# rsinghlab/GNN-Tumor-Seg

Hardware: AMD Instinct MI355X
Metric: supervoxel-graphs/sec training, 7xSAGE-pool-256, 15k-node graphs (higher is better)
Workload: dtype f32; 1 GPU; C2: 7xGraphSAGE-pool-256 (8 SAGEConv), fwd+weighted-CE+bwd+AdamW, 4 x 15000-node/86350-edge lattice graphs per GPU, 4-chan feat, fp32; global_batch=4, nodes_per_batch=60000, edges_per_batch=345400, parallelism=dp1

## Files before the change

### gnn-tumor-seg_amd/csrc/gts_narrow.hip

```cpp
#include "gts_gemm_skinny.h"

namespace gts {
namespace {

constexpr int kFirstW = 256, kFirstS = 4;

__global__ __launch_bounds__(kBlock) void first_layer_bwd_kernel(const float* __restrict__ g, const float* __restrict__ x,
                                                                const float* __restrict__ m0,
                                                                const float* __restrict__ w_neigh, float* __restrict__ gm,
                                                                float* __restrict__ part_x, float* __restrict__ part_m,
                                                                int64_t m, int64_t rows_per_chunk) {
  constexpr int W = kFirstW, S = kFirstS;
  __shared__ v4f red[kWavesPerBlock - 1][2 * S + 1][kWave];
  const int lane = threadIdx.x & (kWave - 1), rl = threadIdx.x / kWave;
  const int64_t row0 = blockIdx.x * rows_per_chunk, row1 = min(m, row0 + rows_per_chunk);
  v4f wn[S];
#pragma unroll
  for (int e = 0; e < 4; ++e) {
    const v4f t = *reinterpret_cast<const v4f*>(w_neigh + static_cast<size_t>(4 * lane + e) * S);
#pragma unroll
    for (int j = 0; j < S; ++j) wn[j][e] = t[j];
  }
  v4f ax[S + 1], am[S];
#pragma unroll
// ... 44 lines not shown
  }
  __syncthreads();
  if (rl != 0) return;
#pragma unroll
  for (int i = 0; i <= S; ++i) {
    v4f total = ax[i];
    for (int l = 1; l < kWavesPerBlock; ++l) total += red[l - 1][i][lane];
    *reinterpret_cast<v4f*>(part_x + (static_cast<size_t>(blockIdx.x) * (S + 1) + i) * W + 4 * lane) = total;
  }
#pragma unroll
  for (int i = 0; i < S; ++i) {
    v4f total = am[i];
    for (int l = 1; l < kWavesPerBlock; ++l) total += red[l - 1][S + 1 + i][lane];
    *reinterpret_cast<v4f*>(part_m + (static_cast<size_t>(blockIdx.x) * S + i) * W + 4 * lane) = total;
  }
}

inline bool first_layer_shape(int64_t m, int64_t w, int64_t s0, int64_t s1) {
  return m > 0 && m < (1LL << 31) && w == kFirstW && s0 == kFirstS && s1 == kFirstS;
}

constexpr int kTopK = 256, kTopC = 4;
constexpr int kCeRowsPerThread = 4, kCeRows = kBlock * kCeRowsPerThread;

__device__ __forceinline__ float top_label_weight(long long label, const float* __restrict__ class_w, bool* valid, int* y) {
  *valid = label >= 0 && label < kTopC;
  *y = *valid ? static_cast<int>(label) : 0;
  return !*valid ? 0.0f : (class_w != nullptr ? class_w[*y] : 1.0f);
}

__global__ __launch_bounds__(kBlock) void top_den_kernel(const int64_t* __restrict__ labels, const float* __restrict__ class_w,
                                                        float* __restrict__ ce_part, int64_t n) {
  __shared__ float red[kWavesPerBlock];
  float den = 0.f;
  const int64_t base = (static_cast<int64_t>(blockIdx.x) * kBlock + threadIdx.x) * kCeRowsPerThread;
  for (int r = 0; r < kCeRowsPerThread; ++r) {
    const int64_t i = base + r;
    if (i >= n) break;
    bool valid;
    int y;
    den += top_label_weight(labels[i], class_w, &valid, &y);
  }
  for (int s = kWave / 2; s >= 1; s >>= 1) den += __shfl_xor(den, s, kWave);
  const int lane = threadIdx.x & (kWave - 1), wave = threadIdx.x / kWave;
  if (lane == 0) red[wave] = den;
  __syncthreads();
  if (threadIdx.x == 0) ce_part[2 * blockIdx.x + 1] = (red[0] + red[1]) + (red[2] + red[3]);
}

__device__ __forceinline__ float lane_value(float v, int lane) {
  return __int_as_float(__builtin_amdgcn_readlane(__float_as_int(v), lane));
}

__global__ __launch_bounds__(kBlock) void top_layer_train_kernel(
    const float* __restrict__ h, const float* __restrict__ mx, const float* __restrict__ w_self,
    const float* __restrict__ w_neigh, const float* __restrict__ bias, const int64_t* __restrict__ labels,
    const float* __restrict__ class_w, const float* __restrict__ ce_part, int ce_blocks, float* __restrict__ logits,
    float* __restrict__ g, float* __restrict__ term, float* __restrict__ part_h, float* __restrict__ part_m,
    float* __restrict__ part_b, int64_t m, int64_t rows_per_chunk) {
  constexpr int W = kTopK, C = kTopC;
  __shared__ v4f red[kWavesPerBlock - 1][2 * C][kWave];
  __shared__ v4f colsum[kBlock];
  __shared__ float dred[kBlock];
  const int lane = threadIdx.x & (kWave - 1), rl = threadIdx.x / kWave;
  const int64_t row0 = blockIdx.x * rows_per_chunk, row1 = min(m, row0 + rows_per_chunk);
  colsum[threadIdx.x] = v4f{0.f, 0.f, 0.f, 0.f};
  float den = 0.f;
  if (ce_part != nullptr) {
    for (int b = threadIdx.x; b < ce_blocks; b += kBlock) den += ce_part[2 * b + 1];
    dred[threadIdx.x] = den;
    __syncthreads();
    for (int s = kBlock / 2; s >= 1; s >>= 1) {
      if (threadIdx.x < s) dred[threadIdx.x] += dred[threadIdx.x + s];
      __syncthreads();
    }
    den = dred[0];
  } else {
    __syncthreads();
  }
  v4f ws[C], wn[C];
#pragma unroll
  for (int n = 0; n < C; ++n) {
    ws[n] = *reinterpret_cast<const v4f*>(w_self + static_cast<size_t>(n) * W + 4 * lane);
    wn[n] = *reinterpret_cast<const v4f*>(w_neigh + static_cast<size_t>(n) * W + 4 * lane);
  }
  const v4f bv = *reinterpret_cast<const v4f*>(bias);
  v4f ah[C], am[C];
#pragma unroll
  for (int i = 0; i < C; ++i) ah[i] = am[i] = v4f{0.f, 0.f, 0.f, 0.f};
  const bool upper32 = (lane & 32) != 0, upper16 = (lane & 16) != 0;
  const int sel = lane & 3;
  auto dots = [&](const v4f fh, const v4f fm) __attribute__((always_inline)) {
    float d[C];
#pragma unroll
    for (int n = 0; n < C; ++n) {
      d[n] = 0.f;
#pragma unroll
      for (int e = 0; e < 4; ++e) d[n] = __builtin_fmaf(fh[e], ws[n][e], d[n]);
#pragma unroll
      for (int e = 0; e < 4; ++e) d[n] = __builtin_fmaf(fm[e], wn[n][e], d[n]);
    }
    const float keep0 = upper32 ? d[2] : d[0], keep1 = upper32 ? d[3] : d[1];
    const float send0 = upper32 ? d[0] : d[2], send1 = upper32 ? d[1] : d[3];
    const float a = keep0 + __shfl_xor(send0, 32, kWave), b = keep1 + __shfl_xor(send1, 32, kWave);
    float c = (upper16 ? b : a) + __shfl_xor(upper16 ? a : b, 16, kWave);
#pragma unroll
    for (int o = 8; o > 0; o >>= 1) c += __shfl_xor(c, o, kWave);
    return c;
  };
  constexpr int kAhead = 4;
  for (int64_t first = row0 + rl; first < row1; first += kAhead * kWavesPerBlock) {
    v4f fh[kAhead], fm[kAhead];
#pragma unroll
    for (int u = 0; u < kAhead; ++u) {
      const int64_t row = first + u * kWavesPerBlock < row1 ? first + u * kWavesPerBlock : first;
      fh[u] = *reinterpret_cast<const v4f*>(h + static_cast<size_t>(row) * W + 4 * lane);
      fm[u] = *reinterpret_cast<const v4f*>(mx + static_cast<size_t>(row) * W + 4 * lane);
    }
    const bool mine = first + sel * kWavesPerBlock < row1;
    const int64_t my_row = mine ? first + sel * kWavesPerBlock : first;
    const long long label = labels[my_row];
    float x[C];
#pragma unroll
    for (int n = 0; n < C; ++n) x[n] = 0.f;
#pragma unroll
    for (int u = 0; u < kAhead; ++u) {
      const float c = dots(fh[u], fm[u]);
#pragma unroll
      for (int n = 0; n < C; ++n) {
        const float t = lane_value(c, 16 * n);
        x[n] = sel == u ? t : x[n];
      }
    }
#pragma unroll
    for (int n = 0; n < C; ++n) x[n] = x[n] + bv[n];
    float v[C];
    float top = -INFINITY;
#pragma unroll
    for (int c = 0; c < C; ++c) v[c] = x[c], top = fmaxf(top, v[c]);
    float sum = 0.f;
#pragma unroll
    for (int c = 0; c < C; ++c) v[c] = expf(v[c] - top), sum += v[c];
    bool valid;
    int y;
    const float w = top_label_weight(label, class_w, &valid, &y);
    const float xy = y == 0 ? x[0] : y == 1 ? x[1] : y == 2 ? x[2] : x[3];
    const float loss_term = valid ? w * (logf(sum) + top - xy) : (label == -100 ? 0.0f : NAN);
    v4f gv;
#pragma unroll
    for (int c = 0; c < C; ++c) {
      const float gu = w * (v[c] / sum - (c == y ? 1.0f : 0.0f));
      gv[c] = ce_part != nullptr ? gu / den : gu;
    }
    if (lane < kAhead && mine) {
      *reinterpret_cast<v4f*>(logits + static_cast<size_t>(my_row) * C) = v4f{x[0], x[1], x[2], x[3]};
      *reinterpret_cast<v4f*>(g + static_cast<size_t>(my_row) * C) = gv;
      term[my_row] = loss_term;
      const int slot = static_cast<int>((my_row - row0) & (kBlock - 1));
      colsum[slot] += 1.0f * gv;
    }
#pragma unroll
    for (int u = 0; u < kAhead; ++u) {
      if (first + u * kWavesPerBlock < row1) {
#pragma unroll
        for (int i = 0; i < C; ++i) {
          const float s = lane_value(gv[i], u);
          ah[i] += s * fh[u];
          am[i] += s * fm[u];
        }
      }
    }
  }
  if (rl > 0) {
#pragma unroll
    for (int i = 0; i < C; ++i) red[rl - 1][i][lane] = ah[i], red[rl - 1][C + i][lane] = am[i];
  }
  __syncthreads();
  if (rl != 0) return;
#pragma unroll
  for (int i = 0; i < C; ++i) {
    v4f total = ah[i];
    for (int l = 1; l < kWavesPerBlock; ++l) total += red[l - 1][i][lane];
    *reinterpret_cast<v4f*>(part_h + (static_cast<size_t>(blockIdx.x) * C + i) * W + 4 * lane) = total;
  }
#pragma unroll
  for (int i = 0; i < C; ++i) {
    v4f total = am[i];
    for (int l = 1; l < kWavesPerBlock; ++l) total += red[l - 1][C + i][lane];
    *reinterpret_cast<v4f*>(part_m + (static_cast<size_t>(blockIdx.x) * C + i) * W + 4 * lane) = total;
  }
  if (lane == 0) {
    const int live = static_cast<int>(min(static_cast<int64_t>(kBlock), row1 - row0));
    v4f total = colsum[0];
    for (int l = 1; l < live; ++l) total += colsum[l];
    *reinterpret_cast<v4f*>(part_b + static_cast<size_t>(blockIdx.x) * C) = total;
  }
}

__global__ __launch_bounds__(kBlock) void top_loss_kernel(const float* __restrict__ term, float* __restrict__ ce_part, int64_t n) {
  __shared__ float red[kWavesPerBlock];
  float num = 0.f;
  const int64_t base = (static_cast<int64_t>(blockIdx.x) * kBlock + threadIdx.x) * kCeRowsPerThread;
  if (base + kCeRowsPerThread <= n) {
    const v4f t = *reinterpret_cast<const v4f*>(term + base);
#pragma unroll
    for (int r = 0; r < kCeRowsPerThread; ++r) num += t[r];
  } else {
    for (int r = 0; r < kCeRowsPerThread; ++r) {
      if (base + r >= n) break;
      num += term[base + r];
    }
  }
  for (int s = kWave / 2; s >= 1; s >>= 1) num += __shfl_xor(num, s, kWave);
  const int lane = threadIdx.x & (kWave - 1), wave = threadIdx.x / kWave;
  if (lane == 0) red[wave] = num;
  __syncthreads();
  if (threadIdx.x == 0) ce_part[2 * blockIdx.x] = (red[0] + red[1]) + (red[2] + red[3]);
}

constexpr int kTopSumGroups = kTopC * kTopK / 16;

__global__ __launch_bounds__(kBlock) void top_finish_kernel(const float* __restrict__ part_h, const float* __restrict__ part_m,
// ... 62 lines not shown
  return t;
}

}
}

extern "C" int64_t gts_sage_first_layer_bwd_workspace(int64_t m, int64_t w, int64_t s0, int64_t s1) {
  using namespace gts;
  if (!first_layer_shape(m, w, s0, s1)) return 0;
  return static_cast<int64_t>(kSkinnyChunks) * (s0 + 1 + s1) * w * static_cast<int64_t>(sizeof(float));
}

extern "C" int32_t gts_sage_first_layer_bwd_f32(const float* g, const float* x, const float* m0, const float* w_neigh,
                                                float* gm, float* gw_self, float* g_bias, float* gw_neigh,
                                                float* workspace, int64_t workspace_bytes, int64_t m, int64_t w,
                                                int64_t s0, int64_t s1, void* stream) {
  using namespace gts;
  if (!g || !x || !m0 || !w_neigh || !gm || !gw_self || !g_bias || !gw_neigh || !workspace) return GTS_ERR_NULL;
  if (!first_layer_shape(m, w, s0, s1)) return GTS_ERR_SHAPE;
  if (workspace_bytes < gts_sage_first_layer_bwd_workspace(m, w, s0, s1)) return GTS_ERR_SHAPE;
  hipStream_t st = static_cast<hipStream_t>(stream);
  const int64_t rpc = (m + kSkinnyChunks - 1) / kSkinnyChunks;
  const int chunks = static_cast<int>((m + rpc - 1) / rpc);
  const int W = kFirstW, S = kFirstS;
  float* part_x = workspace;
  float* part_m = workspace + static_cast<size_t>(chunks) * (S + 1) * W;
  first_layer_bwd_kernel<<<chunks, kBlock, 0, st>>>(g, x, m0, w_neigh, gm, part_x, part_m, m, rpc);
  skinny_sum_kernel<<<((S + 1) * W + 15) / 16, kBlock, 0, st>>>(part_x, gw_self, g_bias, S + 1, S, W, chunks, 1);
  skinny_sum_kernel<<<(S * W + 15) / 16, kBlock, 0, st>>>(part_m, gw_neigh, nullptr, S, S, W, chunks, 1);
  return launch_status();
}

extern "C" int64_t gts_sage_top_layer_train_workspace(int64_t m, int64_t k, int64_t n_classes) {
  using namespace gts;
  if (!top_layer_shape(m, k, n_classes)) return 0;
  return top_workspace(m).total * static_cast<int64_t>(sizeof(float));
}

extern "C" int32_t gts_sage_top_layer_train_f32(const float* h, const float* mx, const float* w_self, const float* w_neigh,
                                                const float* bias, const int64_t* labels, const float* class_w,
                                                int32_t normalise, float* logits, float* g, float* gw_self, float* gw_neigh,
                                                float* g_bias, float* out3, float* workspace, int64_t workspace_bytes,
                                                int64_t m, int64_t k, int64_t n_classes, void* stream) {
  using namespace gts;
  if (!h || !mx || !w_self || !w_neigh || !bias || !labels || !logits || !g || !gw_self || !gw_neigh || !g_bias || !out3 ||
      !workspace)
    return GTS_ERR_NULL;
  if (!top_layer_shape(m, k, n_classes)) return GTS_ERR_SHAPE;
  if (workspace_bytes < gts_sage_top_layer_train_workspace(m, k, n_classes)) return GTS_ERR_SHAPE;
  hipStream_t st = static_cast<hipStream_t>(stream);
  const TopWorkspace t = top_workspace(m);
  float* ce_part = workspace + t.ce_part;
  top_den_kernel<<<t.ce_blocks, kBlock, 0, st>>>(labels, class_w, ce_part, m);
  top_layer_train_kernel<<<t.chunks, kBlock, 0, st>>>(h, mx, w_self, w_neigh, bias, labels, class_w,
                                                     normalise ? ce_part : nullptr, t.ce_blocks, logits, g,
                                                     workspace + t.term, workspace + t.part_h, workspace + t.part_m,
                                                     workspace + t.part_b, m, t.rows_per_chunk);
  top_loss_kernel<<<t.ce_blocks, kBlock, 0, st>>>(workspace + t.term, ce_part, m);
  top_finish_kernel<<<2 * kTopSumGroups + 2, kBlock, 0, st>>>(workspace + t.part_h, workspace + t.part_m, workspace + t.part_b,
                                                             ce_part, gw_self, gw_neigh, g_bias, out3, t.chunks, t.ce_blocks);
  return launch_status();
}
```

### gnn-tumor-seg_amd/csrc/gts_stack.hip

```cpp
#include <algorithm>
#include <vector>

#include "gts_gemm_args.h"

namespace {

constexpr int kMaxLayers = 64;

inline int64_t align256(int64_t bytes) { return (bytes + 255) & ~255LL; }

inline bool bad_stack(int64_t n_rows, const int64_t* widths, int32_t n_layers) {
  if (!widths || n_layers < 1 || n_layers > kMaxLayers || n_rows < 0 || n_rows >= (1LL << 31)) return true;
  for (int i = 0; i <= n_layers; ++i)
    if (widths[i] <= 0 || widths[i] % 4 != 0 || widths[i] >= (1 << 20)) return true;
  return false;
}

struct FwdPlan {
  int64_t m[kMaxLayers], arg[kMaxLayers], out[kMaxLayers], bits[kMaxLayers];
  int64_t p[2];
  int64_t wp[kMaxLayers][3];
  int64_t counters;
  int64_t total;
};
// ... 138 lines not shown
                      int32_t sched_rows, int32_t sched_srcs, int32_t sched_loc_words, const float* x,
                      const float* const* params, int64_t n_rows, const int64_t* widths, int32_t n_layers, int32_t training,
                      int32_t arg_bytes, int32_t relu_bits, void* arena, int64_t arena_bytes, const TopTurn* top,
                      void* stream) {
  if (!indptr || !x || !params || !arena) return GTS_ERR_NULL;
  if (bad_stack(n_rows, widths, n_layers)) return GTS_ERR_SHAPE;
  if (training && arg_bytes != 1 && arg_bytes != 4) return GTS_ERR_ARGKIND;
  for (int i = 0; i < 5 * n_layers; ++i)
    if (!params[i]) return GTS_ERR_NULL;
  const bool train = training != 0;
  const FwdPlan plan = plan_forward(n_rows, widths, n_layers, train, arg_bytes, relu_bits != 0);
  if (arena_bytes < plan.total) return GTS_ERR_SHAPE;
  if (top != nullptr) {
    if (!top->labels || !top->g_top || !top->grads || !top->out3 || !top->workspace) return GTS_ERR_NULL;
    const int64_t need = gts_sage_top_layer_train_workspace(n_rows, widths[n_layers - 1], widths[n_layers]);
    if (need == 0 || top->workspace_bytes < need) return GTS_ERR_SHAPE;
    for (int q = 2; q < 5; ++q)
      if (!top->grads[5 * (n_layers - 1) + q]) return GTS_ERR_NULL;
  }
  if (n_rows == 0) return GTS_OK;
  char* base = static_cast<char*>(arena);
  auto f32 = [&](int64_t off) { return reinterpret_cast<float*>(base + off); };
  uint32_t* counters;
  GTS_TRY(zero_counters(sched_rec, sched_clusters, sched_rows, sched_srcs, sched_loc_words, 0, base + plan.counters, stream, &counters));
  {
    ByShape packs;
    for (int i = 0; i < n_layers; ++i)
      for (int q = 0; q < 3; ++q)
        if (plan.wp[i][q] >= 0)
          packs.add(weight_rows(widths, i, q), widths[i], params[5 * i + kWeightSlot[q]], nullptr, f32(plan.wp[i][q]), nullptr);
    for (const auto& b : packs.groups)
      GTS_TRY(gts_pack_weights_f32(b.in[0].data(), b.out[0].data(), nullptr, b.count(), b.rows, b.cols, 0, stream));
  }
  auto wp = [&](int i, int q) -> const float* { return plan.wp[i][q] >= 0 ? f32(plan.wp[i][q]) : nullptr; };
  const float* h = x;
  float* p = nullptr;
  int cur = 0;
  for (int i = 0; i < n_layers; ++i) {
    const float* w_pool = params[5 * i];
    const float* b_pool = params[5 * i + 1];
    const float* w_self = params[5 * i + 2];
    const float* w_neigh = params[5 * i + 3];
    const float* bias = params[5 * i + 4];
    const int64_t fin = widths[i], fout = widths[i + 1];
    const bool last = i == n_layers - 1;
    if (p == nullptr) {
      p = f32(plan.p[cur]);
      const float* packed[2] = {wp(i, 0), nullptr};
      GTS_TRY(gts_linear_fwd_f32(h, w_pool, nullptr, nullptr, b_pool, p, n_rows, fin, fin, 0, 1, nullptr, packed, stream));
    }
    float* m = f32(plan.m[i]);
    void* arg = train ? static_cast<void*>(base + plan.arg[i]) : nullptr;
    const int ab = train ? arg_bytes : 0;
    if (sched_rec != nullptr && fin == 256 && ab != 4 && n_rows * 1024 < (1LL << 32)) {
      GTS_TRY(gts_spmm_max_fwd_cluster_f32(sched_rec, sched_clusters, sched_rows, sched_srcs, sched_loc_words, p, m, arg, ab,
                                           1, n_rows, fin, counters, stream));
    } else {
      GTS_TRY(gts_spmm_max_fwd_f32(indptr, indices, p, m, arg, ab, 1, n_rows, fin, stream));
    }
    uint64_t* bits = plan.bits[i] >= 0 ? reinterpret_cast<uint64_t*>(base + plan.bits[i]) : nullptr;
    float* out = f32(plan.out[i]);
    if (!last && chainable(fout, fin, fin, fout)) {
      float* p_next = f32(plan.p[cur ^ 1]);
      const float* packed[3] = {wp(i, 1), wp(i, 2), wp(i + 1, 0)};
      GTS_TRY(gts_linear_fwd_chain_f32(h, w_self, m, w_neigh, bias, out, params[5 * (i + 1)], params[5 * (i + 1) + 1], p_next,
                                       n_rows, fout, fin, fin, 1, fout, 1, bits, packed, stream));
      p = p_next, cur ^= 1;
    } else if (last && top != nullptr) {
      float* const* gr = top->grads + 5 * i;
      GTS_TRY(gts_sage_top_layer_train_f32(h, m, w_self, w_neigh, bias, top->labels, top->class_w, top->normalise, out,
                                           top->g_top, gr[2], gr[3], gr[4], top->out3, top->workspace, top->workspace_bytes,
                                           n_rows, fin, fout, stream));
      p = nullptr;
    } else {
      const float* packed[2] = {wp(i, 1), wp(i, 2)};
      GTS_TRY(gts_linear_fwd_f32(h, w_self, m, w_neigh, bias, out, n_rows, fout, fin, fin, last ? 0 : 1, bits, packed, stream));
      p = nullptr;
    }
    h = out;
  }
  return GTS_OK;
}

}

extern "C" int32_t gts_sage_pool_stack_fwd_f32(const int32_t* indptr, const int32_t* indices, const int32_t* sched_rec,
                                               int64_t sched_clusters, int32_t sched_rows, int32_t sched_srcs,
                                               int32_t sched_loc_words, const float* x, const float* const* params,
                                               int64_t n_rows, const int64_t* widths, int32_t n_layers, int32_t training,
                                               int32_t arg_bytes, int32_t relu_bits, void* arena, int64_t arena_bytes,
                                               void* stream) {
  return stack_forward(indptr, indices, sched_rec, sched_clusters, sched_rows, sched_srcs, sched_loc_words, x, params, n_rows,
                       widths, n_layers, training, arg_bytes, relu_bits, arena, arena_bytes, nullptr, stream);
}

extern "C" int32_t gts_sage_pool_stack_train_fwd_f32(const int32_t* indptr, const int32_t* indices, const int32_t* sched_rec,
                                                     int64_t sched_clusters, int32_t sched_rows, int32_t sched_srcs,
                                                     int32_t sched_loc_words, const float* x, const float* const* params,
                                                     int64_t n_rows, const int64_t* widths, int32_t n_layers,
                                                     int32_t arg_bytes, int32_t relu_bits, void* arena, int64_t arena_bytes,
                                                     const int64_t* labels, const float* class_w, int32_t normalise,
                                                     float* g_top, float* const* grads, float* out3, float* top_workspace,
                                                     int64_t top_workspace_bytes, void* stream) {
  const TopTurn top{labels, class_w, normalise, g_top, grads, out3, top_workspace, top_workspace_bytes};
  return stack_forward(indptr, indices, sched_rec, sched_clusters, sched_rows, sched_srcs, sched_loc_words, x, params, n_rows,
                       widths, n_layers, 1, arg_bytes, relu_bits, arena, arena_bytes, &top, stream);
}

extern "C" int64_t gts_sage_pool_stack_bwd_scratch(int64_t n_rows, const int64_t* widths, int32_t n_layers,
                                                   int32_t ) {
  if (bad_stack(n_rows, widths, n_layers)) return -1;
  return plan_backward(n_rows, widths, n_layers).total;
}

extern "C" int32_t gts_sage_pool_stack_bwd_f32(const int32_t* t_indptr, const int32_t* t_indices, const int32_t* t_slot,
                                               const int32_t* sched_rec, int64_t sched_clusters, int32_t sched_rows,
                                               int32_t sched_srcs, int32_t sched_loc_words, const float* gout, const float* x,
                                               const float* const* params, int64_t n_rows, const int64_t* widths,
                                               int32_t n_layers, int32_t arg_bytes, int32_t relu_bits, const void* fwd_arena,
                                               float* const* grads, float* gx, void* scratch, int64_t scratch_bytes,
                                               void* stream) {
  return gts_sage_pool_stack_bwd_top_f32(t_indptr, t_indices, t_slot, sched_rec, sched_clusters, sched_rows, sched_srcs,
                                         sched_loc_words, gout, x, params, n_rows, widths, n_layers, arg_bytes, relu_bits,
                                         fwd_arena, grads, gx, scratch, scratch_bytes, 0, stream);
}
// ... 127 lines not shown
```

### gnn-tumor-seg_amd/gts/dense.py

```python
import torch
import torch.nn.functional as F

from . import _lib
from ._lib import check, current_stream, ptr, require_device
from ._operands import StreamBuffers, f32

GEMM_TIMER = None
_OPT_GEMM_TILE = _lib.const("GTS_OPT_GEMM_TILE")


class row_count_invariant:

    _depth = 0
    _saved = -1
    _lock = __import__("threading").Lock()

    def __enter__(self):
        with row_count_invariant._lock:
            if row_count_invariant._depth == 0:
                lib = _lib.load()
                row_count_invariant._saved = int(lib.gts_get_option(_OPT_GEMM_TILE))
                check(lib.gts_set_option(_OPT_GEMM_TILE, -2), "gts_set_option")
            row_count_invariant._depth += 1
        return self
# ... 333 lines not shown
                                          arr(*[ptr(t) for t in gws]), arr(*[ptr(t) for t in gbs]), q,
                                          ptr(ws), ws.numel() * 4, m, n_p, k_p, current_stream()),
            "gts_linear_bwd_weight_f32"))
    out = []
    for gw, gb in zip(gws, gbs):
        if (n_p, k_p) != (n, k):
            gw = gw[:n, :k].contiguous()
            gb = gb[:n].contiguous() if gb is not None else None
        out.append((gw, gb))
    return out


def linear_bwd_weight(g, a, want_bias_grad=False):
    return linear_bwd_weight_multi([(g, a, want_bias_grad)])[0]


def first_layer_bwd_applies(g, x, m0, w_neigh):
    return g.shape[0] > 0 and g.shape[1] == 256 and x.shape[1] == 4 and m0.shape[1] == 4 and tuple(w_neigh.shape) == (256, 4)


def sage_first_layer_bwd(g, x, m0, w_neigh):
    if not first_layer_bwd_applies(_mat(g, "g"), _mat(x, "x"), _mat(m0, "m0"), _mat(w_neigh, "w_neigh")):
        raise _lib.GtsError("sage_first_layer_bwd takes g [M, 256], x [M, 4], m0 [M, 4], w_neigh [256, 4] with M > 0")
    _same(x.shape[0], g.shape[0], "rows of g / x")
    _same(m0.shape[0], g.shape[0], "rows of g / m0")
    g, x, m0, w_neigh = _dense(g, x, m0, w_neigh)
    dev = _operands(g, x, m0, w_neigh)
    m = g.shape[0]
    gm = torch.empty((m, 4), dtype=torch.float32, device=dev)
    gw_self, gw_neigh = (torch.empty((256, 4), dtype=torch.float32, device=dev) for _ in range(2))
    g_bias = torch.empty(256, dtype=torch.float32, device=dev)
    lib = _lib.load()
    nbytes = lib.gts_sage_first_layer_bwd_workspace(m, 256, 4, 4)
    ws = _gemm_ws.get(dev, nbytes)
    check(lib.gts_sage_first_layer_bwd_f32(ptr(g), ptr(x), ptr(m0), ptr(w_neigh), ptr(gm), ptr(gw_self), ptr(g_bias),
                                           ptr(gw_neigh), ptr(ws), ws.numel() * 4, m, 256, 4, 4, current_stream()),
          "gts_sage_first_layer_bwd_f32")
    return gm, gw_self, g_bias, gw_neigh


def top_layer_train_applies(h, m, w_self, w_neigh):
    return h.shape[0] > 0 and h.shape[1] == 256 and m.shape[1] == 256 and tuple(w_self.shape) == (4, 256) \
        and tuple(w_neigh.shape) == (4, 256)


_top_ws = StreamBuffers()


def top_layer_train_workspace(rows, device):
    nbytes = _lib.load().gts_sage_top_layer_train_workspace(rows, 256, 4)
    return _top_ws.get(device, nbytes), nbytes


def sage_top_layer_train(h, m, w_self, w_neigh, bias, labels, class_w=None, normalise=True, out=None):
    if not top_layer_train_applies(_mat(h, "h"), _mat(m, "m"), _mat(w_self, "w_self"), _mat(w_neigh, "w_neigh")):
        raise _lib.GtsError("sage_top_layer_train takes h [M, 256], m [M, 256], w_self [4, 256], w_neigh [4, 256] with M > 0")
    _same(m.shape[0], h.shape[0], "rows of h / m")
    h, m, w_self, w_neigh, bias = _dense(h, m, w_self, w_neigh, bias)
    dev = _operands(h, m, w_self, w_neigh, bias, class_w)
    rows = h.shape[0]
    if tuple(bias.shape) != (4,) or (class_w is not None and tuple(class_w.shape) != (4,)):
        raise _lib.GtsError("sage_top_layer_train takes bias [4] and class weights [4]")
    if labels.dtype != torch.int64 or tuple(labels.shape) != (rows,) or not labels.is_contiguous() or labels.device != dev:
        raise _lib.GtsError(f"labels must be contiguous int64 [{rows}] on {dev}")
    logits, g = (torch.empty((rows, 4), dtype=torch.float32, device=dev) for _ in range(2))
    if out is None:
        out = (torch.empty((4, 256), dtype=torch.float32, device=dev), torch.empty((4, 256), dtype=torch.float32, device=dev),
               torch.empty(4, dtype=torch.float32, device=dev))
    gw_self, gw_neigh, g_bias = out
    stats = torch.empty(3, dtype=torch.float32, device=dev)
    ws, nbytes = top_layer_train_workspace(rows, dev)
    check(_lib.load().gts_sage_top_layer_train_f32(
        ptr(h), ptr(m), ptr(w_self), ptr(w_neigh), ptr(bias), ptr(labels), ptr(class_w), 1 if normalise else 0, ptr(logits),
        ptr(g), ptr(gw_self), ptr(gw_neigh), ptr(g_bias), ptr(stats), ptr(ws), ws.numel() * 4, rows, 256, 4,
        current_stream()), "gts_sage_top_layer_train_f32")
    return logits, g, gw_self, gw_neigh, g_bias, stats


def relu_bwd(g, out):
    return g * (out > 0)


class _Linear(torch.autograd.Function):

    @staticmethod
    def forward(ctx, x, w, bias):
        ctx.save_for_backward(x, w)
        ctx.has_bias = bias is not None
        return linear_fwd(x, w, bias=bias)

    @staticmethod
    def backward(ctx, gy):
        x, w = ctx.saved_tensors
        gy = gy.contiguous()
        gx = linear_bwd_input(gy, w) if ctx.needs_input_grad[0] else None
        gw = gb = None
        if ctx.needs_input_grad[1] or (ctx.has_bias and ctx.needs_input_grad[2]):
            gw, gb = linear_bwd_weight(gy, x, want_bias_grad=ctx.has_bias)
        return gx, gw, gb if ctx.has_bias else None


def linear(x, w, bias=None):
    return _Linear.apply(x, w, bias)
```

### gnn-tumor-seg_amd/gts/nn.py

```python
import os

import torch
import torch.nn as nn
import torch.nn.functional as F

from . import dense, ops
from .graph import _DeviceSchedule


class GraphError(RuntimeError):
    """Counterpart of dgl.DGLError for the checks the layers make."""


def _is_relu(fn):
    return fn in (F.relu, torch.relu, torch.nn.functional.relu)


class _SagePoolLayer(torch.autograd.Function):

    @staticmethod
    def forward(ctx, g, h, w_pool, b_pool, w_self, w_neigh, bias, relu_out, need_bwd):
        h = h.contiguous()
        p = dense.linear_fwd(h, w_pool, bias=b_pool, relu=True)
        m, arg = ops.spmm_max_fwd(g, p, want_arg=need_bwd, relu_input=True)
# ... 84 lines not shown
    if key not in _identities:
        _identities[key] = torch.eye(n, dtype=torch.float32, device=device)
    return _identities[key]


RELU_MASK_BITS = os.environ.get("GTS_RELU_BITS", "1") != "0"


def _chainable(a0, w0, a1, w2):
    n, k0, k1, n2 = w0.shape[0], a0.shape[1], a1.shape[1], w2.shape[0]
    return n % 4 == 0 and k0 % 4 == 0 and k1 % 4 == 0 and n <= 256 and n2 <= 256 and w2.shape[1] == n


def _pool_layer_weight_grads(g, gp, h, m, w_pool, w_self):
    if w_pool.shape == w_self.shape:
        (g_ws, g_bias), (g_wn, _), (g_wp, g_bp) = dense.linear_bwd_weight_multi(
            [(g, h, True), (g, m, False), (gp, h, True)])
    else:
        (g_ws, g_bias), (g_wn, _) = dense.linear_bwd_weight_multi([(g, h, True), (g, m, False)])
        g_wp, g_bp = dense.linear_bwd_weight(gp, h, want_bias_grad=True)
    return g_ws, g_wn, g_wp, g_bias, g_bp


def _pack_by_shape(weights, transposed, want_plain=False):
    by_shape, plain, fragment = {}, {}, {}
    for w in weights:
        by_shape.setdefault(tuple(w.shape), []).append(w)
    for ws in by_shape.values():
        copies = dense.pack_weights(ws, transposed=transposed, want_plain=want_plain)
        if want_plain:
            plain.update((id(w), wt) for w, wt in zip(ws, copies[0]))
            copies = copies[1]
        fragment.update((id(w), wp) for w, wp in zip(ws, copies))
    return (plain, fragment) if want_plain else fragment


class _SagePoolStack(torch.autograd.Function):

    @staticmethod
    def launch_forward(g, x, need_bwd, params, top=None):
        n_layers = len(params) // 5
        h = x.contiguous()
        saved = []
        turn = None
        hbits = None
        p = None
        fragment = _pack_by_shape([w for i in range(n_layers) for w in (params[5 * i], params[5 * i + 2], params[5 * i + 3])
                                   if w.shape[0] > 128 and w.shape[1] % 4 == 0], transposed=False)
        for i in range(n_layers):
            w_pool, b_pool, w_self, w_neigh, bias = params[5 * i:5 * i + 5]
            last = i == n_layers - 1
            if p is None:
                p = dense.linear_fwd(h, w_pool, bias=b_pool, relu=True, packed=(fragment.get(id(w_pool)), None))
            m, arg = ops.spmm_max_fwd(g, p, want_arg=need_bwd, relu_input=True)
            p = None
            nxt = params[5 * (i + 1):5 * (i + 1) + 2] if not last else None
            obits = dense.relu_bits_empty(h.shape[0], w_self.shape[0], h.device) \
                if RELU_MASK_BITS and need_bwd and not last and dense.relu_bits_pay(h.shape[0], w_self.shape[0]) else None
            if nxt is not None and _chainable(h, w_self, m, nxt[0]):
                out, p = dense.linear_fwd_chain(h, w_self, m, w_neigh, bias, True, nxt[0], nxt[1], True, relu_bits=obits,
                                                packed=(fragment.get(id(w_self)), fragment.get(id(w_neigh)), fragment.get(id(nxt[0]))))
            elif last and top is not None:
                labels, class_w, normalise, dst = top
                out, *turn = dense.sage_top_layer_train(h, m, w_self, w_neigh, bias, labels, class_w, normalise, out=dst)
            else:
                out = dense.linear_fwd(h, w_self, m, w_neigh, bias=bias, relu=not last, relu_bits=obits,
                                       packed=(fragment.get(id(w_self)), fragment.get(id(w_neigh))))
            saved += [h, m, arg, hbits]
            h, hbits = out, obits
        return h, saved, turn

    @staticmethod
    def forward(ctx, g, x, need_bwd, *params):
        h, saved, _ = _SagePoolStack.launch_forward(g, x, need_bwd, params)
        if need_bwd:
            ctx.g, ctx.n_layers = g, len(params) // 5
            ctx.save_for_backward(*saved, *params)
        return h

    @staticmethod
    def backward(ctx, gout):
        n = ctx.n_layers
        tensors = ctx.saved_tensors
        gx, grads = _SagePoolStack.launch_backward(ctx.g, tensors[:4 * n], tensors[4 * n:], gout, ctx.needs_input_grad[1])
        return (None, gx, None, *grads)

    @staticmethod
    def launch_backward(graph, acts, params, gout, need_gx, top_done=False):
        n = len(params) // 5
        grads = [None] * (5 * n)
        g = gout.contiguous()
        gx = None
        deferred = {}

        turned, turned_fragment = _pack_by_shape(
            [w for w in (params[5 * i + j] for i in range(n) for j in (0, 2, 3))
             if w.shape[1] >= 128 and w.shape[0] % 4 == 0 and w.shape[1] % 4 == 0], transposed=True, want_plain=True)

        def igrad(g0, w0, g1=None, w1=None, relu_mask=None, relu_bits=None):
            if id(w0) in turned and (w1 is None or id(w1) in turned) and g0.is_contiguous():
                return dense.linear_bwd_input_t(g0, turned[id(w0)], g1, turned[id(w1)] if w1 is not None else None,
                                                relu_mask=relu_mask, relu_bits=relu_bits,
                                                packed=(turned_fragment[id(w0)], turned_fragment[id(w1)] if w1 is not None else None))
            return dense.linear_bwd_input(g0, w0, g1, w1, relu_mask=relu_mask)

        def defer(grad_out, act, slot, bias_slot):
# ... 521 lines not shown
```

### include/gts_hip.h

```cpp
#ifndef GTS_HIP_H
#define GTS_HIP_H

#include <stdint.h>

#ifdef __cplusplus
extern "C" {
#endif

#define GTS_OK 0
#define GTS_ERR_NULL (-1)
#define GTS_ERR_SHAPE (-2)
#define GTS_ERR_ARGKIND (-3)

int32_t gts_abi_version(void);
const char* gts_error_string(int32_t code);

int32_t gts_spmm_max_fwd_f32(const int32_t* indptr, const int32_t* indices, const float* x,
                             float* out, void* arg, int32_t arg_bytes, int32_t relu_input,
                             int64_t n_dst, int64_t n_feat, void* stream);

int32_t gts_spmm_max_bwd_f32(const int32_t* t_indptr, const int32_t* t_indices,
                             const int32_t* t_slot, const float* gout, const void* arg,
                             int32_t arg_bytes, const float* relu_src, float* gx,
                             int64_t n_src, int64_t n_feat, void* stream);
// ... 108 lines not shown

int64_t gts_relu_bits_bytes(int64_t m, int64_t n);
int32_t gts_relu_bits_pay(int64_t m, int64_t n);
int32_t gts_linear_fwd_f32(const float* a0, const float* w0, const float* a1, const float* w1,
                           const float* bias, float* out, int64_t m, int64_t n, int64_t k0,
                           int64_t k1, int32_t relu, uint64_t* relu_bits, const float* const* packed,
                           void* stream);
int64_t gts_packed_weight_floats(int64_t n, int64_t k);
int32_t gts_pack_weights_f32(const float* const* src, float* const* dst, float* const* plain_t, int32_t n_mats,
                             int64_t rows, int64_t cols, int32_t transposed, void* stream);
int32_t gts_linear_bwd_input_f32(const float* g0, const float* w0, const float* g1, const float* w1,
                                 const float* relu_mask, float* gin, int64_t m, int64_t k,
                                 int64_t n0, int64_t n1, void* stream);
int32_t gts_linear_bwd_input_t_f32(const float* g0, const float* w0t, const float* g1, const float* w1t,
                                   const float* relu_mask, const uint64_t* relu_bits, float* gin, int64_t m,
                                   int64_t k, int64_t n0, int64_t n1, const float* const* packed, void* stream);
int64_t gts_linear_bwd_input_t_act_workspace(int64_t m, int64_t k);
int32_t gts_linear_bwd_input_t_act_f32(const float* g0, const float* w0t, const float* g1, const float* w1t,
                                       const float* act_out, int32_t activation, float* gin, float* g_bias,
                                       float* workspace, int64_t workspace_bytes, int64_t m, int64_t k,
                                       int64_t n0, int64_t n1, const float* const* packed,
                                       void* stream);
int64_t gts_gat_fc_scores_workspace(int64_t m, int64_t heads, int64_t dim);
int32_t gts_gat_fc_scores_f32(const float* h, const float* w_fc, const float* attn_l, const float* attn_r,
                              float* ft, float* el, float* er, float* workspace, int64_t workspace_bytes,
                              int64_t m, int64_t heads, int64_t dim, int64_t k, const float* w_fc_packed, void* stream);
int32_t gts_linear_fwd_chain_f32(const float* a0, const float* w0, const float* a1, const float* w1,
                                 const float* bias, float* out, const float* w2, const float* bias2,
                                 float* out2, int64_t m, int64_t n, int64_t k0, int64_t k1, int32_t relu,
                                 int64_t n2, int32_t relu2, uint64_t* relu_bits, const float* const* packed,
                                 void* stream);
int32_t gts_linear_bwd_input_chain_t_f32(const float* g0, const float* w0t, const float* g1,
                                         const float* w1t, const float* relu_mask, const uint64_t* relu_bits,
                                         float* gin, const float* w2t, float* gin2, int64_t m, int64_t k,
                                         int64_t n0, int64_t n1, int64_t k2, const float* const* packed,
                                         void* stream);
int32_t gts_transpose_batch_f32(const float* const* src, float* const* dst, int32_t n_mats,
                                int64_t rows, int64_t cols, void* stream);
int64_t gts_linear_bwd_weight_workspace(int64_t m, int64_t n, int64_t k, int32_t n_problems);
int32_t gts_linear_bwd_weight_f32(const float* const* g, const float* const* a, float* const* gw,
                                  float* const* gb, int32_t n_problems, float* workspace,
                                  int64_t workspace_bytes, int64_t m, int64_t n, int64_t k,
                                  void* stream);
int64_t gts_sage_first_layer_bwd_workspace(int64_t m, int64_t w, int64_t s0, int64_t s1);
int32_t gts_sage_first_layer_bwd_f32(const float* g, const float* x, const float* m0, const float* w_neigh, float* gm,
                                     float* gw_self, float* g_bias, float* gw_neigh, float* workspace,
                                     int64_t workspace_bytes, int64_t m, int64_t w, int64_t s0, int64_t s1, void* stream);
int64_t gts_sage_top_layer_train_workspace(int64_t m, int64_t k, int64_t n_classes);
int32_t gts_sage_top_layer_train_f32(const float* h, const float* mx, const float* w_self, const float* w_neigh,
                                     const float* bias, const int64_t* labels, const float* class_w, int32_t normalise,
                                     float* logits, float* g, float* gw_self, float* gw_neigh, float* g_bias, float* out3,
                                     float* workspace, int64_t workspace_bytes, int64_t m, int64_t k, int64_t n_classes,
                                     void* stream);

int64_t gts_sage_pool_stack_fwd_arena(int64_t n_rows, const int64_t* widths, int32_t n_layers, int32_t training,
                                      int32_t arg_bytes, int32_t relu_bits, int64_t* offsets);
int32_t gts_sage_pool_stack_fwd_f32(const int32_t* indptr, const int32_t* indices, const int32_t* sched_rec,
                                    int64_t sched_clusters, int32_t sched_rows, int32_t sched_srcs,
                                    int32_t sched_loc_words, const float* x, const float* const* params,
                                    int64_t n_rows, const int64_t* widths, int32_t n_layers, int32_t training,
                                    int32_t arg_bytes, int32_t relu_bits, void* arena, int64_t arena_bytes, void* stream);
int64_t gts_sage_pool_stack_bwd_scratch(int64_t n_rows, const int64_t* widths, int32_t n_layers, int32_t relu_bits);
int32_t gts_sage_pool_stack_bwd_f32(const int32_t* t_indptr, const int32_t* t_indices, const int32_t* t_slot,
                                    const int32_t* sched_rec, int64_t sched_clusters, int32_t sched_rows,
                                    int32_t sched_srcs, int32_t sched_loc_words, const float* gout, const float* x,
                                    const float* const* params, int64_t n_rows, const int64_t* widths,
                                    int32_t n_layers, int32_t arg_bytes, int32_t relu_bits, const void* fwd_arena,
                                    float* const* grads, float* gx, void* scratch, int64_t scratch_bytes,
                                    void* stream);
int32_t gts_sage_pool_stack_train_fwd_f32(const int32_t* indptr, const int32_t* indices, const int32_t* sched_rec,
                                          int64_t sched_clusters, int32_t sched_rows, int32_t sched_srcs,
                                          int32_t sched_loc_words, const float* x, const float* const* params,
                                          int64_t n_rows, const int64_t* widths, int32_t n_layers, int32_t arg_bytes,
                                          int32_t relu_bits, void* arena, int64_t arena_bytes, const int64_t* labels,
                                          const float* class_w, int32_t normalise, float* g_top, float* const* grads,
                                          float* out3, float* top_workspace, int64_t top_workspace_bytes, void* stream);
int32_t gts_sage_pool_stack_bwd_top_f32(const int32_t* t_indptr, const int32_t* t_indices, const int32_t* t_slot,
                                        const int32_t* sched_rec, int64_t sched_clusters, int32_t sched_rows,
                                        int32_t sched_srcs, int32_t sched_loc_words, const float* gout, const float* x,
                                        const float* const* params, int64_t n_rows, const int64_t* widths,
                                        int32_t n_layers, int32_t arg_bytes, int32_t relu_bits, const void* fwd_arena,
                                        float* const* grads, float* gx, void* scratch, int64_t scratch_bytes,
                                        int32_t top_done, void* stream);

int64_t gts_weighted_ce_workspace(int64_t n);
int32_t gts_weighted_ce_f32(const float* logits, const int64_t* labels, const float* class_w,
                            float* grad_unscaled, float* workspace, int64_t workspace_bytes,
                            float* out3, int64_t n, int64_t n_classes, void* stream);

#define GTS_DICE_CE_MAX_GROUPS 8
#define GTS_DICE_CE_STATS_FLOATS 40
#define GTS_DICE_CE_STATS_LOSS 0
#define GTS_DICE_CE_STATS_CE 1
#define GTS_DICE_CE_STATS_LDICE 2
#define GTS_DICE_CE_STATS_CE_NUM 3
#define GTS_DICE_CE_STATS_CE_DEN 4
#define GTS_DICE_CE_STATS_DICE 8
#define GTS_DICE_CE_STATS_I 16
#define GTS_DICE_CE_STATS_S 24
#define GTS_DICE_CE_STATS_T 32
int64_t gts_dice_ce_workspace(int64_t n, int32_t n_groups);
int32_t gts_dice_ce_fwd_f32(const float* logits, const int64_t* labels, const float* class_w,
                            const uint32_t* group_masks, int32_t n_groups, double ce_weight,
                            double dice_weight, double smooth, float* stats, void* workspace,
                            int64_t workspace_bytes, int64_t n, int64_t n_classes, void* stream);
int32_t gts_dice_ce_bwd_f32(const float* logits, const int64_t* labels, const float* class_w,
// ... 220 lines not shown
```

Before: 983.3 graphs/s.

## Fuse last-layer neighbour max-pool gather into top-layer train kernel

Adds a POOL variant of the top-layer fused train kernel that gathers neighbour rows of the pooled features via CSR and computes the max-aggregation and its argmax bytes inline, instead of first writing the aggregated matrix with a separate SpMM-max kernel. Neighbour loads are software-pipelined across row groups with double buffers. This removes one kernel launch and the write and re-read of an M x 256 aggregated tensor for the last layer. In exchange the top kernel gets more register pressure and irregular gather traffic, and it uses plain CSR rather than the cluster schedule.

```diff
diff --git a/gnn-tumor-seg_amd/csrc/gts_narrow.hip b/gnn-tumor-seg_amd/csrc/gts_narrow.hip
--- a/gnn-tumor-seg_amd/csrc/gts_narrow.hip
+++ b/gnn-tumor-seg_amd/csrc/gts_narrow.hip
@@ -120,11 +120,15 @@
   return __int_as_float(__builtin_amdgcn_readlane(__float_as_int(v), lane));
 }
 
+constexpr int kPoolEdges = 8;
+
+template <bool POOL>
 __global__ __launch_bounds__(kBlock) void top_layer_train_kernel(
-    const float* __restrict__ h, const float* __restrict__ mx, const float* __restrict__ w_self,
-    const float* __restrict__ w_neigh, const float* __restrict__ bias, const int64_t* __restrict__ labels,
-    const float* __restrict__ class_w, const float* __restrict__ ce_part, int ce_blocks, float* __restrict__ logits,
-    float* __restrict__ g, float* __restrict__ term, float* __restrict__ part_h, float* __restrict__ part_m,
+    const int32_t* __restrict__ indptr, const int32_t* __restrict__ indices, const float* __restrict__ h,
+    const float* __restrict__ mx, const float* __restrict__ w_self, const float* __restrict__ w_neigh,
+    const float* __restrict__ bias, const int64_t* __restrict__ labels, const float* __restrict__ class_w,
+    const float* __restrict__ ce_part, int ce_blocks, float* __restrict__ logits, float* __restrict__ g,
+    uint8_t* __restrict__ arg, float* __restrict__ term, float* __restrict__ part_h, float* __restrict__ part_m,
     float* __restrict__ part_b, int64_t m, int64_t rows_per_chunk) {
   constexpr int W = kTopK, C = kTopC;
   __shared__ v4f red[kWavesPerBlock - 1][2 * C][kWave];
@@ -177,17 +181,8 @@
     return c;
   };
   constexpr int kAhead = 4;
-  for (int64_t first = row0 + rl; first < row1; first += kAhead * kWavesPerBlock) {
-    v4f fh[kAhead], fm[kAhead];
-#pragma unroll
-    for (int u = 0; u < kAhead; ++u) {
-      const int64_t row = first + u * kWavesPerBlock < row1 ? first + u * kWavesPerBlock : first;
-      fh[u] = *reinterpret_cast<const v4f*>(h + static_cast<size_t>(row) * W + 4 * lane);
-      fm[u] = *reinterpret_cast<const v4f*>(mx + static_cast<size_t>(row) * W + 4 * lane);
-    }
-    const bool mine = first + sel * kWavesPerBlock < row1;
-    const int64_t my_row = mine ? first + sel * kWavesPerBlock : first;
-    const long long label = labels[my_row];
+  auto finish_group = [&](const int64_t first, const long long label, const bool mine, const int64_t my_row,
+                          const v4f (&fh)[kAhead], const v4f (&fm)[kAhead]) __attribute__((always_inline)) {
     float x[C];
 #pragma unroll
     for (int n = 0; n < C; ++n) x[n] = 0.f;
@@ -236,6 +231,119 @@
           ah[i] += s * fh[u];
           am[i] += s * fm[u];
         }
+      }
+    }
+  };
+  if constexpr (!POOL) {
+    for (int64_t first = row0 + rl; first < row1; first += kAhead * kWavesPerBlock) {
+      v4f fh[kAhead], fm[kAhead];
+#pragma unroll
+      for (int u = 0; u < kAhead; ++u) {
+        const int64_t row = first + u * kWavesPerBlock < row1 ? first + u * kWavesPerBlock : first;
+        fh[u] = *reinterpret_cast<const v4f*>(h + static_cast<size_t>(row) * W + 4 * lane);
+        fm[u] = *reinterpret_cast<const v4f*>(mx + static_cast<size_t>(row) * W + 4 * lane);
+      }
+      const bool mine = first + sel * kWavesPerBlock < row1;
+      const int64_t my_row = mine ? first + sel * kWavesPerBlock : first;
+      finish_group(first, labels[my_row], mine, my_row, fh, fm);
+    }
+  } else {
+    constexpr int kStep = kAhead * kWavesPerBlock;
+    const int64_t start = row0 + rl;
+    auto load_ext = [&](const int64_t first) __attribute__((always_inline)) {
+      const int64_t r = first + (lane & 3) * kWavesPerBlock;
+      return lane < 2 * kAhead && r < row1 ? indptr[r + (lane >> 2)] : 0;
+    };
+    auto load_eid = [&](const int ext) __attribute__((always_inline)) {
+      const int u = (lane >> 3) & 3, j = lane & (kPoolEdges - 1);
+      const int beg = __shfl(ext, u, kWave), end = __shfl(ext, kAhead + u, kWave);
+      return lane < kAhead * kPoolEdges && j < end - beg ? indices[beg + j] : 0;
+    };
+    auto issue = [&](v4f (&buf)[kPoolEdges], const int ext, const int eid, const int u) __attribute__((always_inline)) {
+      const int deg = __builtin_amdgcn_readlane(ext, kAhead + u) - __builtin_amdgcn_readlane(ext, u);
+      const int last = max(min(deg, kPoolEdges) - 1, 0);
+#pragma unroll
+      for (int j = 0; j < kPoolEdges; ++j) {
+        const int src = __builtin_amdgcn_readlane(eid, kPoolEdges * u + min(j, last));
+        buf[j] = *reinterpret_cast<const v4f*>(mx + static_cast<size_t>(src) * W + 4 * lane);
+      }
+    };
+    auto consume = [&](const v4f (&buf)[kPoolEdges], const int ext, const int u, const int64_t row)
+                       __attribute__((always_inline)) {
+      const int beg = __builtin_amdgcn_readlane(ext, u), deg = __builtin_amdgcn_readlane(ext, kAhead + u) - beg;
+      const int last = max(min(deg, kPoolEdges) - 1, 0);
+      float best[4];
+      int slot[4];
+#pragma unroll
+      for (int t = 0; t < 4; ++t) best[t] = -INFINITY, slot[t] = -1;
+#pragma unroll
+      for (int j = 0; j < kPoolEdges; ++j) {
+        const int e = min(j, last);
+#pragma unroll
+        for (int t = 0; t < 4; ++t) {
+          if (best[t] < buf[j][t]) best[t] = buf[j][t], slot[t] = e;
+        }
+      }
+      if (deg <= 0) {
+#pragma unroll
+        for (int t = 0; t < 4; ++t) best[t] = -INFINITY, slot[t] = -1;
+      }
+      for (int k = kPoolEdges; k < deg; k += kPoolEdges) {
+        v4f val[kPoolEdges];
+#pragma unroll
+        for (int j = 0; j < kPoolEdges; ++j) {
+          const int src = indices[beg + min(k + j, deg - 1)];
+          val[j] = *reinterpret_cast<const v4f*>(mx + static_cast<size_t>(src) * W + 4 * lane);
+        }
+#pragma unroll
+        for (int j = 0; j < kPoolEdges; ++j) {
+          const int e = min(k + j, deg - 1);
+#pragma unroll
+          for (int t = 0; t < 4; ++t) {
+            if (best[t] < val[j][t]) best[t] = val[j][t], slot[t] = e;
+          }
+        }
+      }
+      v4f o;
+      uint32_t word = 0;
+#pragma unroll
+      for (int t = 0; t < 4; ++t) {
+        const bool dead = isinf(best[t]);
+        o[t] = dead ? 0.0f : best[t];
+        const uint32_t s = (dead || !(best[t] > 0.0f)) ? 0xFFu : static_cast<uint32_t>(slot[t]) & 0xFFu;
+        word |= s << (8 * t);
+      }
+      if (row < row1) *reinterpret_cast<uint32_t*>(arg + static_cast<size_t>(row) * W + 4 * lane) = word;
+      return o;
+    };
+    if (start < row1) {
+      int ext_cur = load_ext(start), ext_nxt = load_ext(start + kStep);
+      int eid_cur = load_eid(ext_cur);
+      v4f buf_a[kPoolEdges], buf_b[kPoolEdges];
+      issue(buf_a, ext_cur, eid_cur, 0);
+      issue(buf_b, ext_cur, eid_cur, 1);
+      for (int64_t first = start; first < row1; first += kStep) {
+        v4f fh[kAhead], fm[kAhead];
+#pragma unroll
+        for (int u = 0; u < kAhead; ++u) {
+          const int64_t row = first + u * kWavesPerBlock < row1 ? first + u * kWavesPerBlock : first;
+          fh[u] = *reinterpret_cast<const v4f*>(h + static_cast<size_t>(row) * W + 4 * lane);
+        }
+        const bool mine = first + sel * kWavesPerBlock < row1;
+        const int64_t my_row = mine ? first + sel * kWavesPerBlock : first;
+        const long long label = labels[my_row];
+        const int eid_nxt = load_eid(ext_nxt);
+        const int ext_far = load_ext(first + 2 * kStep);
+        fm[0] = consume(buf_a, ext_cur, 0, first);
+        issue(buf_a, ext_cur, eid_cur, 2);
+        fm[1] = consume(buf_b, ext_cur, 1, first + kWavesPerBlock);
+        issue(buf_b, ext_cur, eid_cur, 3);
+        fm[2] = consume(buf_a, ext_cur, 2, first + 2 * kWavesPerBlock);
+        issue(buf_a, ext_nxt, eid_nxt, 0);
+        fm[3] = consume(buf_b, ext_cur, 3, first + 3 * kWavesPerBlock);
+        issue(buf_b, ext_nxt, eid_nxt, 1);
+        finish_group(first, label, mine, my_row, fh, fm);
+        ext_cur = ext_nxt, ext_nxt = ext_far, eid_cur = eid_nxt;
       }
     }
   }
@@ -404,12 +512,45 @@
   const TopWorkspace t = top_workspace(m);
   float* ce_part = workspace + t.ce_part;
   top_den_kernel<<<t.ce_blocks, kBlock, 0, st>>>(labels, class_w, ce_part, m);
-  top_layer_train_kernel<<<t.chunks, kBlock, 0, st>>>(h, mx, w_self, w_neigh, bias, labels, class_w,
-                                                     normalise ? ce_part : nullptr, t.ce_blocks, logits, g,
-                                                     workspace + t.term, workspace + t.part_h, workspace + t.part_m,
-                                                     workspace + t.part_b, m, t.rows_per_chunk);
+  top_layer_train_kernel<false><<<t.chunks, kBlock, 0, st>>>(nullptr, nullptr, h, mx, w_self, w_neigh, bias, labels, class_w,
+                                                            normalise ? ce_part : nullptr, t.ce_blocks, logits, g, nullptr,
+                                                            workspace + t.term, workspace + t.part_h, workspace + t.part_m,
+                                                            workspace + t.part_b, m, t.rows_per_chunk);
   top_loss_kernel<<<t.ce_blocks, kBlock, 0, st>>>(workspace + t.term, ce_part, m);
   top_finish_kernel<<<2 * kTopSumGroups + 2, kBlock, 0, st>>>(workspace + t.part_h, workspace + t.part_m, workspace + t.part_b,
                                                              ce_part, gw_self, gw_neigh, g_bias, out3, t.chunks, t.ce_blocks);
   return launch_status();
 }
+
+extern "C" int64_t gts_sage_top_layer_train_pool_workspace(int64_t m, int64_t k, int64_t n_classes) {
+  return gts_sage_top_layer_train_workspace(m, k, n_classes);
+}
+
+extern "C" int32_t gts_sage_top_layer_train_pool_f32(const int32_t* indptr, const int32_t* indices, const float* h,
+                                                     const float* p, const float* w_self, const float* w_neigh,
+                                                     const float* bias, const int64_t* labels, const float* class_w,
+                                                     int32_t normalise, float* logits, float* g, float* gw_self,
+                                                     float* gw_neigh, float* g_bias, float* out3, void* arg,
+                                                     int32_t arg_bytes, float* workspace, int64_t workspace_bytes, int64_t m,
+                                                     int64_t k, int64_t n_classes, void* stream) {
+  using namespace gts;
+  if (!indptr || !h || !p || !w_self || !w_neigh || !bias || !labels || !logits || !g || !gw_self || !gw_neigh || !g_bias ||
+      !out3 || !arg || !workspace)
+    return GTS_ERR_NULL;
+  if (arg_bytes != 1) return GTS_ERR_ARGKIND;
+  if (!top_layer_shape(m, k, n_classes)) return GTS_ERR_SHAPE;
+  if (workspace_bytes < gts_sage_top_layer_train_pool_workspace(m, k, n_classes)) return GTS_ERR_SHAPE;
+  hipStream_t st = static_cast<hipStream_t>(stream);
+  const TopWorkspace t = top_workspace(m);
+  float* ce_part = workspace + t.ce_part;
+  top_den_kernel<<<t.ce_blocks, kBlock, 0, st>>>(labels, class_w, ce_part, m);
+  top_layer_train_kernel<true><<<t.chunks, kBlock, 0, st>>>(indptr, indices, h, p, w_self, w_neigh, bias, labels, class_w,
+                                                           normalise ? ce_part : nullptr, t.ce_blocks, logits, g,
+                                                           static_cast<uint8_t*>(arg), workspace + t.term,
+                                                           workspace + t.part_h, workspace + t.part_m, workspace + t.part_b, m,
+                                                           t.rows_per_chunk);
+  top_loss_kernel<<<t.ce_blocks, kBlock, 0, st>>>(workspace + t.term, ce_part, m);
+  top_finish_kernel<<<2 * kTopSumGroups + 2, kBlock, 0, st>>>(workspace + t.part_h, workspace + t.part_m, workspace + t.part_b,
+                                                             ce_part, gw_self, gw_neigh, g_bias, out3, t.chunks, t.ce_blocks);
+  return launch_status();
+}
diff --git a/gnn-tumor-seg_amd/csrc/gts_stack.hip b/gnn-tumor-seg_amd/csrc/gts_stack.hip
--- a/gnn-tumor-seg_amd/csrc/gts_stack.hip
+++ b/gnn-tumor-seg_amd/csrc/gts_stack.hip
@@ -214,7 +214,9 @@
     float* m = f32(plan.m[i]);
     void* arg = train ? static_cast<void*>(base + plan.arg[i]) : nullptr;
     const int ab = train ? arg_bytes : 0;
-    if (sched_rec != nullptr && fin == 256 && ab != 4 && n_rows * 1024 < (1LL << 32)) {
+    const bool top_pools = last && top != nullptr && ab == 1;
+    if (top_pools) {
+    } else if (sched_rec != nullptr && fin == 256 && ab != 4 && n_rows * 1024 < (1LL << 32)) {
       GTS_TRY(gts_spmm_max_fwd_cluster_f32(sched_rec, sched_clusters, sched_rows, sched_srcs, sched_loc_words, p, m, arg, ab,
                                            1, n_rows, fin, counters, stream));
     } else {
@@ -230,9 +232,14 @@
       p = p_next, cur ^= 1;
     } else if (last && top != nullptr) {
       float* const* gr = top->grads + 5 * i;
-      GTS_TRY(gts_sage_top_layer_train_f32(h, m, w_self, w_neigh, bias, top->labels, top->class_w, top->normalise, out,
-                                           top->g_top, gr[2], gr[3], gr[4], top->out3, top->workspace, top->workspace_bytes,
-                                           n_rows, fin, fout, stream));
+      if (top_pools)
+        GTS_TRY(gts_sage_top_layer_train_pool_f32(indptr, indices, h, p, w_self, w_neigh, bias, top->labels, top->class_w,
+                                                  top->normalise, out, top->g_top, gr[2], gr[3], gr[4], top->out3, arg, ab,
+                                                  top->workspace, top->workspace_bytes, n_rows, fin, fout, stream));
+      else
+        GTS_TRY(gts_sage_top_layer_train_f32(h, m, w_self, w_neigh, bias, top->labels, top->class_w, top->normalise, out,
+                                             top->g_top, gr[2], gr[3], gr[4], top->out3, top->workspace, top->workspace_bytes,
+                                             n_rows, fin, fout, stream));
       p = nullptr;
     } else {
       const float* packed[2] = {wp(i, 1), wp(i, 2)};
diff --git a/gnn-tumor-seg_amd/gts/dense.py b/gnn-tumor-seg_amd/gts/dense.py
--- a/gnn-tumor-seg_amd/gts/dense.py
+++ b/gnn-tumor-seg_amd/gts/dense.py
@@ -409,7 +409,7 @@
     return _top_ws.get(device, nbytes), nbytes
 
 
-def sage_top_layer_train(h, m, w_self, w_neigh, bias, labels, class_w=None, normalise=True, out=None):
+def sage_top_layer_train(h, m, w_self, w_neigh, bias, labels, class_w=None, normalise=True, out=None, pool=None):
     if not top_layer_train_applies(_mat(h, "h"), _mat(m, "m"), _mat(w_self, "w_self"), _mat(w_neigh, "w_neigh")):
         raise _lib.GtsError("sage_top_layer_train takes h [M, 256], m [M, 256], w_self [4, 256], w_neigh [4, 256] with M > 0")
     _same(m.shape[0], h.shape[0], "rows of h / m")
@@ -420,6 +420,12 @@
         raise _lib.GtsError("sage_top_layer_train takes bias [4] and class weights [4]")
     if labels.dtype != torch.int64 or tuple(labels.shape) != (rows,) or not labels.is_contiguous() or labels.device != dev:
         raise _lib.GtsError(f"labels must be contiguous int64 [{rows}] on {dev}")
+    if pool is not None:
+        indptr, indices = pool
+        for name, t in (("indptr", indptr), ("indices", indices)):
+            if t.dtype != torch.int32 or t.dim() != 1 or not t.is_contiguous() or t.device != dev:
+                raise _lib.GtsError(f"{name} must be a contiguous int32 vector on {dev}")
+        _same(indptr.numel(), rows + 1, "entries of indptr / rows + 1")
     logits, g = (torch.empty((rows, 4), dtype=torch.float32, device=dev) for _ in range(2))
     if out is None:
         out = (torch.empty((4, 256), dtype=torch.float32, device=dev), torch.empty((4, 256), dtype=torch.float32, device=dev),
@@ -427,11 +433,18 @@
     gw_self, gw_neigh, g_bias = out
     stats = torch.empty(3, dtype=torch.float32, device=dev)
     ws, nbytes = top_layer_train_workspace(rows, dev)
-    check(_lib.load().gts_sage_top_layer_train_f32(
-        ptr(h), ptr(m), ptr(w_self), ptr(w_neigh), ptr(bias), ptr(labels), ptr(class_w), 1 if normalise else 0, ptr(logits),
-        ptr(g), ptr(gw_self), ptr(gw_neigh), ptr(g_bias), ptr(stats), ptr(ws), ws.numel() * 4, rows, 256, 4,
-        current_stream()), "gts_sage_top_layer_train_f32")
-    return logits, g, gw_self, gw_neigh, g_bias, stats
+    if pool is None:
+        check(_lib.load().gts_sage_top_layer_train_f32(
+            ptr(h), ptr(m), ptr(w_self), ptr(w_neigh), ptr(bias), ptr(labels), ptr(class_w), 1 if normalise else 0, ptr(logits),
+            ptr(g), ptr(gw_self), ptr(gw_neigh), ptr(g_bias), ptr(stats), ptr(ws), ws.numel() * 4, rows, 256, 4,
+            current_stream()), "gts_sage_top_layer_train_f32")
+        return logits, g, gw_self, gw_neigh, g_bias, stats
+    arg = torch.empty((rows, 256), dtype=torch.uint8, device=dev)
+    check(_lib.load().gts_sage_top_layer_train_pool_f32(
+        ptr(indptr), ptr(indices), ptr(h), ptr(m), ptr(w_self), ptr(w_neigh), ptr(bias), ptr(labels), ptr(class_w),
+        1 if normalise else 0, ptr(logits), ptr(g), ptr(gw_self), ptr(gw_neigh), ptr(g_bias), ptr(stats), ptr(arg), 1, ptr(ws),
+        ws.numel() * 4, rows, 256, 4, current_stream()), "gts_sage_top_layer_train_pool_f32")
+    return logits, g, gw_self, gw_neigh, g_bias, stats, arg
 
 
 def relu_bwd(g, out):
diff --git a/gnn-tumor-seg_amd/gts/nn.py b/gnn-tumor-seg_amd/gts/nn.py
--- a/gnn-tumor-seg_amd/gts/nn.py
+++ b/gnn-tumor-seg_amd/gts/nn.py
@@ -160,6 +160,15 @@
             last = i == n_layers - 1
             if p is None:
                 p = dense.linear_fwd(h, w_pool, bias=b_pool, relu=True, packed=(fragment.get(id(w_pool)), None))
+            top_pools = last and top is not None and need_bwd and g.arg_bytes == 1
+            if top_pools:
+                labels, class_w, normalise, dst = top
+                d = g.dev()
+                out, *turn, arg = dense.sage_top_layer_train(h, p, w_self, w_neigh, bias, labels, class_w, normalise, out=dst,
+                                                             pool=(d.indptr, d.indices))
+                saved += [h, None, arg, hbits]
+                h, hbits = out, None
+                break
             m, arg = ops.spmm_max_fwd(g, p, want_arg=need_bwd, relu_input=True)
             p = None
             nxt = params[5 * (i + 1):5 * (i + 1) + 2] if not last else None
diff --git a/include/gts_hip.h b/include/gts_hip.h
--- a/include/gts_hip.h
+++ b/include/gts_hip.h
@@ -184,6 +184,13 @@
                                      float* logits, float* g, float* gw_self, float* gw_neigh, float* g_bias, float* out3,
                                      float* workspace, int64_t workspace_bytes, int64_t m, int64_t k, int64_t n_classes,
                                      void* stream);
+int64_t gts_sage_top_layer_train_pool_workspace(int64_t m, int64_t k, int64_t n_classes);
+int32_t gts_sage_top_layer_train_pool_f32(const int32_t* indptr, const int32_t* indices, const float* h, const float* p,
+                                          const float* w_self, const float* w_neigh, const float* bias,
+                                          const int64_t* labels, const float* class_w, int32_t normalise, float* logits,
+                                          float* g, float* gw_self, float* gw_neigh, float* g_bias, float* out3, void* arg,
+                                          int32_t arg_bytes, float* workspace, int64_t workspace_bytes, int64_t m, int64_t k,
+                                          int64_t n_classes, void* stream);
 
 int64_t gts_sage_pool_stack_fwd_arena(int64_t n_rows, const int64_t* widths, int32_t n_layers, int32_t training,
                                       int32_t arg_bytes, int32_t relu_bits, int64_t* offsets);
```

Measured after the change: 979.6 graphs/s. Within noise of the previous version (-0.4%).
